# MolecularAI/GraphINVENT

Hardware: NVIDIA B200
Metric: molecular-graphs/sec (train fwd+bwd) GGNN (higher is better)
Workload: dtype f32

## Files before the change

graphinvent_b200/csrc/gemm.cuh:

```cuda
#pragma once
#include "common.cuh"
#include "prof.cuh"

namespace gib {

enum Epi : int {
  EPI_ACT = 0,
  EPI_MUL_DACT = 1,
  EPI_ADD = 2
};

struct GemmNT {
  const float* A = nullptr; int lda = 0;
  const float* B = nullptr; int ldb = 0;
  const float* B_hi = nullptr;
  const float* B_lo = nullptr;
  float* C = nullptr; int ldc = 0;
  int M = 0, N = 0, K = 0;
  const float* bias = nullptr;
  int act = ACT_NONE;
  int mode = EPI_ACT;
  const float* aux = nullptr; int ldaux = 0;
  int n_store = 0;
  int n_valid = 0;
  double work = 0;
  const int* m_dev = nullptr;
  const int* base_dev = nullptr;
};

struct GemmTN {
  const float* G; int ldg;
  const float* X; int ldx;
  int M, Nn, Kk, chunk_rows;
  float* ws; float* ws_bias;
};

struct GemmDW {
  const float* G = nullptr; int ldg = 0; int Nn = 0;
  const float* X = nullptr; int ldx = 0; int Kk = 0;
  int M = 0;
  float* dW = nullptr; float* dbias = nullptr;
  int R = 0, C = 0, Rb = 0, Rbp = 0;
  long long rs = 0, cs = 1;
  float* scratch = nullptr;
  size_t half_floats = 0;
  double work = 0;
  const int* m_dev = nullptr;
  const int* base_dev = nullptr;
};

constexpr int kTc3MaxProblems = 16;

struct Dw3Layout {
  int chunk_rows;
  int cap_splits[kTc3MaxProblems];
  size_t part_off[kTc3MaxProblems];
  size_t bias_off[kTc3MaxProblems];
  size_t floats;
};

int gemm_nt(const GemmNT& p, cudaStream_t st);
int gemm_nt_simt(const GemmNT& p, cudaStream_t st);
int gemm_nt_tc(const GemmNT& p, cudaStream_t st);
int gemm_nt_tc_group(const GemmNT* ps, int n, cudaStream_t st);
int gemm_nt_group(const GemmNT* ps, int n, cudaStream_t st);
bool gemm_nt_chain_ok(const GemmNT* ps, int n);
int gemm_nt_chain(const GemmNT* ps, const int* dep, int n, int* flags, cudaStream_t st);
bool tc_eligible(const GemmNT& p);
bool tc3_eligible(const GemmNT& p);
int gemm_nt_tc3_group(const GemmNT* ps, int n, cudaStream_t st);
size_t tc3_chain_flag_ints(const GemmNT* ps, int n);
int gemm_nt_tc3_chain(const GemmNT* ps, const int* dep, int n, int* flags, cudaStream_t st);
bool tc3_dw_eligible(const GemmDW& q);
int tc3_dw_chunk_rows(const GemmDW* qs, int n, long long plan_rows);
void tc3_dw_layout(const GemmDW* qs, int n, int chunk_rows, Dw3Layout* L);
int gemm_dw_tc3_partials(const GemmDW* qs, int n, const Dw3Layout& L, float* scratch, cudaStream_t st);
int gemm_dw_tc3_reduce(const GemmDW* qs, int n, const Dw3Layout& L, const float* scratch, cudaStream_t st);
int device_sm_count();
void tc3_set_trace(long long* buf, int tiles);
int tc_make_map(void* cu_tensor_map, const float* base, int rows, int cols, int ld, int box_rows, int mn_major);
extern bool g_use_tc;
extern int g_tc_debug;
extern long long* g_tc_timing;

enum tc_timing_slots {
  TS_TMA_WAIT_EMPTY = 0, TS_TMA_TOTAL, TS_MMA_WAIT_SPLIT, TS_MMA_WAIT_ACC, TS_MMA_TOTAL, TS_SPL_WAIT_RAW, TS_SPL_WORK,
  TS_SPL_TOTAL, TS_EPI_WAIT_ACC, TS_EPI_WORK, TS_EPI_TOTAL, TS_KERNEL_TOTAL, TS_ITEMS, TS_KBLOCKS, TS_LAUNCHES,
  TIMING_SLOTS = 16, TIMING_CTAS = 160
};

int gemm_dw(const GemmDW& q, cudaStream_t st);
int gemm_dw_group(const GemmDW* qs, int n, long long plan_rows, cudaStream_t st);
size_t gemm_dw_group_half_floats(const GemmDW* qs, int n, long long plan_rows);
int dw_begin();
void gemm_dw_plan(int M, int Nn, int Kk, int* splits, int* chunk);
void tc_dw_plan(int M, int Nn, int Kk, int* splits, int* chunk);
bool tc_dw_eligible(const GemmDW& q);
int gemm_dw_tc_partials(const GemmDW& q, int* splits_out, cudaStream_t st);
size_t gemm_dw_scratch_floats(int M, int Nn, int Kk);
size_t gemm_dw_half_floats(int M, int Nn, int Kk);
int dw_join(cudaStream_t st);

}
```

graphinvent_b200/csrc/gemm_simt.cu:

```cuda
#include <algorithm>
#include <mutex>

#include "gemm.cuh"
#include "ops.cuh"

namespace gib {

constexpr int BK = 16;
constexpr int kColsumSplits = 296;

template <int BM, int BN, int RM, int RN>
__global__ void __launch_bounds__(256, 2) sgemm_nt_kernel(const GemmNT p) {
  static_assert((BM / (4 * RM)) * (BN / (4 * RN)) == 256, "256 threads");
  __shared__ __align__(16) float As[2][BK][BM + 4];
  __shared__ __align__(16) float Bs[2][BK][BN + 4];

  const int tid = threadIdx.x;
  const int w = tid >> 5, l = tid & 31;
  const int ty = (w >> 1) * 4 + (l >> 3);
  const int tx = (w & 1) * 8 + (l & 7);
  const int m0 = blockIdx.y * BM, n0 = blockIdx.x * BN;

  constexpr int LA = BM / 64, LB = BN / 64;
  float4 ra[LA], rb[LB];
// ... 76 lines not shown
    }
    if (t + 1 < ntiles) sstore(buf ^ 1);
    __syncthreads();
  }

  const bool vec_c = (p.ldc & 3) == 0 && ((reinterpret_cast<uintptr_t>(p.C) & 15) == 0);
  const bool vec_x = p.aux && (p.ldaux & 3) == 0 && ((reinterpret_cast<uintptr_t>(p.aux) & 15) == 0);
#pragma unroll
  for (int a = 0; a < RM; ++a)
#pragma unroll
    for (int i = 0; i < 4; ++i) {
      const int m = m0 + ty * 4 + a * (BM / RM) + i;
      if (m >= p.M) continue;
#pragma unroll
      for (int b = 0; b < RN; ++b) {
        const int n = n0 + tx * 4 + b * (BN / RN);
        if (n >= p.n_store) continue;
        float v[4] = {acc[a][i][b][0], acc[a][i][b][1], acc[a][i][b][2], acc[a][i][b][3]};
        float x[4] = {0.f, 0.f, 0.f, 0.f};
        if (p.mode != EPI_ACT) {
          if (vec_x && n + 3 < p.n_store) {
            float4 t4 = *reinterpret_cast<const float4*>(p.aux + (size_t)m * p.ldaux + n);
            x[0] = t4.x; x[1] = t4.y; x[2] = t4.z; x[3] = t4.w;
          } else {
#pragma unroll
            for (int j = 0; j < 4; ++j)
              if (n + j < p.n_store) x[j] = p.aux[(size_t)m * p.ldaux + n + j];
          }
        }
#pragma unroll
        for (int j = 0; j < 4; ++j) {
          if (p.mode == EPI_ACT) {
            float bj = (p.bias && n + j < p.N) ? p.bias[n + j] : 0.f;
            v[j] = act_f(v[j] + bj, p.act);
          } else if (p.mode == EPI_MUL_DACT) {
            v[j] = v[j] * dact_from_out(x[j], p.act);
          } else {
            v[j] = v[j] + x[j];
          }
          if (n + j >= p.n_valid) v[j] = 0.f;
        }
        float* dst = p.C + (size_t)m * p.ldc + n;
        if (vec_c && n + 3 < p.n_store) {
          *reinterpret_cast<float4*>(dst) = make_float4(v[0], v[1], v[2], v[3]);
        } else {
#pragma unroll
          for (int j = 0; j < 4; ++j)
            if (n + j < p.n_store) dst[j] = v[j];
        }
      }
    }
}

static inline bool use_tc3() { return (g_tc_debug & 1) == 0; }

int gemm_nt(const GemmNT& p, cudaStream_t st) {
  if (p.m_dev) {
    if (!g_use_tc || !use_tc3() || !tc3_eligible(p)) {
      set_error("gemm_nt: device-side row counts need the tcgen05 path (tensor cores on, pre-split weights)");
      return -2;
    }
    return gemm_nt_tc3_group(&p, 1, st);
  }
  if (g_use_tc && p.N >= 48 && p.K >= 32) {
    if (use_tc3() && p.M >= 256 && tc3_eligible(p)) return gemm_nt_tc3_group(&p, 1, st);
    if (p.M >= 1024 && tc_eligible(p)) return gemm_nt_tc(p, st);
  }
  if (g_use_tc && use_tc3() && (g_tc_debug & 4) && p.N < 48 && p.K >= 128 && p.M >= 256 && tc3_eligible(p))
    return gemm_nt_tc3_group(&p, 1, st);
  return gemm_nt_simt(p, st);
}

int gemm_nt_group(const GemmNT* ps, int n, cudaStream_t st) {
  if (n == 1) return gemm_nt(ps[0], st);
  bool ok = g_use_tc && n <= 4, ok3 = ok && use_tc3(), dyn = false;
  long long tiles = 0;
  for (int i = 0; i < n && ok; ++i) {
    if (ps[i].m_dev) dyn = true;
    if (ps[i].M <= 0 || ps[i].N <= 0) continue;
    ok = tc_eligible(ps[i]) && ps[i].K >= 32 && ps[i].N >= 48;
    ok3 = ok3 && ok && tc3_eligible(ps[i]);
    tiles += (long long)ceil_div(ps[i].M, 128) * ceil_div(ps[i].N, 128);
  }
  if (ok3 && (tiles >= 4 || dyn)) return gemm_nt_tc3_group(ps, n, st);
  if (ok && !dyn && tiles >= 16) return gemm_nt_tc_group(ps, n, st);
  for (int i = 0; i < n; ++i) GIB_TRY(gemm_nt(ps[i], st));
  return 0;
}

bool gemm_nt_chain_ok(const GemmNT* ps, int n) {
  if (!g_use_tc || !use_tc3() || n < 2 || n > kTc3MaxProblems || (g_tc_debug & 2)) return false;
  long long tiles = 0;
  bool dyn = false;
  for (int i = 0; i < n; ++i) {
    const GemmNT& p = ps[i];
    if (p.M <= 0 || p.N <= 0) continue;
    if (!tc3_eligible(p) || p.N < 48 || p.K < 32) return false;
    if (p.m_dev) dyn = true;
    tiles += (long long)ceil_div(p.M, 128) * ceil_div(p.N, 128);
  }
  return dyn || tiles >= 16;
}
int gemm_nt_chain(const GemmNT* ps, const int* dep, int n, int* flags, cudaStream_t st) {
  return gemm_nt_tc3_chain(ps, dep, n, flags, st);
}

int gemm_nt_simt(const GemmNT& p, cudaStream_t st) {
  if (p.M <= 0 || p.N <= 0) return 0;
  if (p.K % BK != 0 || (p.lda & 3) || (p.ldb & 3) || p.K <= 0) {
    set_error("gemm_nt: K=%d lda=%d ldb=%d violate the padded-layout contract", p.K, p.lda, p.ldb);
    return -2;
  }
  ProfScope prof(PROF_GEMM_NT_SIMT, p.work > 0 ? p.work : 2.0 * p.M * (double)p.N * p.K, st);
  const long long ctas_big = (long long)ceil_div(p.M, 128) * ceil_div(p.N, 128);
  const int num_sms = device_sm_count();
  if (ctas_big >= num_sms && p.N > 64) {
    dim3 grid(ceil_div(p.N, 128), ceil_div(p.M, 128));
    sgemm_nt_kernel<128, 128, 2, 2><<<grid, 256, 0, st>>>(p);
  } else if (p.N <= 64 && (long long)ceil_div(p.M, 128) >= num_sms) {
    dim3 grid(ceil_div(p.N, 64), ceil_div(p.M, 128));
    sgemm_nt_kernel<128, 64, 2, 1><<<grid, 256, 0, st>>>(p);
  } else {
    dim3 grid(ceil_div(p.N, 64), ceil_div(p.M, 64));
    sgemm_nt_kernel<64, 64, 1, 1><<<grid, 256, 0, st>>>(p);
  }
  GIB_LAUNCH_CHECK();
  return 0;
}

template <int BM, int BN, int RM, int RN>
__global__ void __launch_bounds__(256, 2) sgemm_tn_splitk_kernel(const GemmTN p) {
  __shared__ __align__(16) float As[2][BK][BM + 4];
  __shared__ __align__(16) float Bs[2][BK][BN + 4];
  const int tid = threadIdx.x;
  const int w = tid >> 5, l = tid & 31;
  const int ty = (w >> 1) * 4 + (l >> 3);
  const int tx = (w & 1) * 8 + (l & 7);
  const int n0 = blockIdx.y * BM;
  const int k0 = blockIdx.x * BN;
  const int z = blockIdx.z;
  const int m_begin = z * p.chunk_rows;
  const int m_end = min(p.M, m_begin + p.chunk_rows);

  constexpr int LA = BM / 64, LB = BN / 64;
  float4 ra[LA], rb[LB];
  auto gload = [&](int m0) {
#pragma unroll
    for (int i = 0; i < LA; ++i) {
      int q = tid + i * 256, kk = q / (BM / 4), c = (q % (BM / 4)) * 4;
      bool ok = (m0 + kk) < m_end && (n0 + c) < p.Nn;
      ra[i] = ok ? __ldg(reinterpret_cast<const float4*>(p.G + (size_t)(m0 + kk) * p.ldg + n0 + c))
                 : make_float4(0, 0, 0, 0);
    }
#pragma unroll
    for (int i = 0; i < LB; ++i) {
      int q = tid + i * 256, kk = q / (BN / 4), c = (q % (BN / 4)) * 4;
      bool ok = (m0 + kk) < m_end && (k0 + c) < p.Kk;
      rb[i] = ok ? __ldg(reinterpret_cast<const float4*>(p.X + (size_t)(m0 + kk) * p.ldx + k0 + c))
                 : make_float4(0, 0, 0, 0);
    }
  };
  auto sstore = [&](int buf) {
#pragma unroll
    for (int i = 0; i < LA; ++i) {
      int q = tid + i * 256, kk = q / (BM / 4), c = (q % (BM / 4)) * 4;
      *reinterpret_cast<float4*>(&As[buf][kk][c]) = ra[i];
    }
#pragma unroll
    for (int i = 0; i < LB; ++i) {
// ... 21 lines not shown
    gload(m_begin);
    sstore(0);
  }
  __syncthreads();
  for (int t = 0; t < ntiles; ++t) {
    const int buf = t & 1;
    if (t + 1 < ntiles) gload(m_begin + (t + 1) * BK);
#pragma unroll
    for (int kk = 0; kk < BK; ++kk) {
      float4 fa[RM], fb[RN];
#pragma unroll
      for (int a = 0; a < RM; ++a)
        fa[a] = *reinterpret_cast<const float4*>(&As[buf][kk][ty * 4 + a * (BM / RM)]);
#pragma unroll
      for (int b = 0; b < RN; ++b)
        fb[b] = *reinterpret_cast<const float4*>(&Bs[buf][kk][tx * 4 + b * (BN / RN)]);
#pragma unroll
      for (int a = 0; a < RM; ++a) {
        const float av[4] = {fa[a].x, fa[a].y, fa[a].z, fa[a].w};
        if (do_bias) {
#pragma unroll
          for (int i = 0; i < 4; ++i) bacc[a][i] += av[i];
        }
#pragma unroll
        for (int b = 0; b < RN; ++b) {
          const float bv[4] = {fb[b].x, fb[b].y, fb[b].z, fb[b].w};
#pragma unroll
          for (int i = 0; i < 4; ++i)
#pragma unroll
            for (int j = 0; j < 4; ++j) acc[a][i][b][j] = fmaf(av[i], bv[j], acc[a][i][b][j]);
        }
      }
    }
    if (t + 1 < ntiles) sstore(buf ^ 1);
    __syncthreads();
  }

  float* out = p.ws + (size_t)z * p.Nn * p.Kk;
#pragma unroll
  for (int a = 0; a < RM; ++a)
#pragma unroll
    for (int i = 0; i < 4; ++i) {
      const int n = n0 + ty * 4 + a * (BM / RM) + i;
      if (n >= p.Nn) continue;
#pragma unroll
      for (int b = 0; b < RN; ++b) {
        const int k = k0 + tx * 4 + b * (BN / RN);
        if (k >= p.Kk) continue;
        *reinterpret_cast<float4*>(out + (size_t)n * p.Kk + k) =
            make_float4(acc[a][i][b][0], acc[a][i][b][1], acc[a][i][b][2], acc[a][i][b][3]);
      }
      if (do_bias && (l & 7) == 0) p.ws_bias[(size_t)z * p.Nn + n] = bacc[a][i];
    }
}

__global__ void __launch_bounds__(256) reduce_grads_kernel(const float* __restrict__ ws, int splits, int Nn, int Kk,
                                                           float* __restrict__ dW, int R, int C, int Rb, int Rbp,
                                                           long long rs, long long cs, int nblk_w,
                                                           const float* __restrict__ wsb, int bsplits,
                                                           float* __restrict__ db) {
  if ((int)blockIdx.x < nblk_w) {
    const long long idx = (long long)blockIdx.x * 256 + threadIdx.x;
    if (idx >= (long long)R * C) return;
    const int r = (int)(idx / C), c = (int)(idx % C);
    const int prow = (r / Rb) * Rbp + (r % Rb);
    const float* src = ws + (size_t)prow * Kk + c;
    const size_t stride = (size_t)Nn * Kk;
    float s = 0.f;
    int zi = 0;
    for (; zi + 8 <= splits; zi += 8) {
      float v[8];
#pragma unroll
      for (int u = 0; u < 8; ++u) v[u] = src[(size_t)(zi + u) * stride];
#pragma unroll
      for (int u = 0; u < 8; ++u) s += v[u];
    }
    for (; zi < splits; ++zi) s += src[(size_t)zi * stride];
    dW[r * rs + c * cs] += s;
  } else {
    __shared__ float sm[8][33];
    const int r = ((int)blockIdx.x - nblk_w) * 32 + (threadIdx.x & 31);
    const int wy = threadIdx.x >> 5;
    float s = 0.f;
    if (r < R) {
      const int prow = (r / Rb) * Rbp + (r % Rb);
      for (int zi = wy; zi < bsplits; zi += 8) s += wsb[(size_t)zi * Nn + prow];
    }
    sm[wy][threadIdx.x & 31] = s;
    __syncthreads();
    if (wy == 0 && r < R) {
      float t = 0.f;
      for (int k = 0; k < 8; ++k) t += sm[k][threadIdx.x];
      db[r] += t;
    }
  }
}

static int launch_reduce(const float* ws, int splits, const GemmDW& q, const float* wsb, int bsplits, cudaStream_t st) {
  const int nblk_w = q.dW ? (int)ceil_div_ll((long long)q.R * q.C, 256) : 0;
  const int nblk_b = q.dbias ? ceil_div(q.R, 32) : 0;
  if (nblk_w + nblk_b == 0) return 0;
  reduce_grads_kernel<<<nblk_w + nblk_b, 256, 0, st>>>(ws, splits, q.Nn, q.Kk, q.dW, q.R, q.C, q.Rb, q.Rbp, q.rs, q.cs,
                                                      nblk_w, wsb, bsplits, q.dbias);
  GIB_LAUNCH_CHECK();
  return 0;
}
// ... 39 lines not shown
}

struct DwSide {
  cudaStream_t side = nullptr;
  cudaEvent_t ev_tn[2], ev_done[2];
  bool done_valid[2] = {false, false};
  long long calls = 0;
  int pending = -1;
  int last = -1;
};
static DwSide g_dw[64];
static std::mutex g_dw_mu;

static int dw_side(DwSide** out) {
  int dev = 0;
  GIB_CUDA_TRY(cudaGetDevice(&dev));
  if (dev < 0 || dev >= 64) { set_error("device index %d out of range", dev); return -4; }
  std::lock_guard<std::mutex> lk(g_dw_mu);
  DwSide& d = g_dw[dev];
  if (!d.side) {
    GIB_CUDA_TRY(cudaStreamCreateWithFlags(&d.side, cudaStreamNonBlocking));
    for (int i = 0; i < 2; ++i) {
      GIB_CUDA_TRY(cudaEventCreateWithFlags(&d.ev_tn[i], cudaEventDisableTiming));
      GIB_CUDA_TRY(cudaEventCreateWithFlags(&d.ev_done[i], cudaEventDisableTiming));
    }
  }
  *out = &d;
  return 0;
}

int dw_begin() {
  DwSide* d;
  GIB_TRY(dw_side(&d));
  d->done_valid[0] = d->done_valid[1] = false;
  d->calls = 0; d->pending = -1; d->last = -1;
  return 0;
}

int dw_join(cudaStream_t st) {
  DwSide* d;
  GIB_TRY(dw_side(&d));
  if (d->last >= 0) {
    GIB_CUDA_TRY(cudaStreamWaitEvent(st, d->ev_done[d->last], 0));
    d->last = -1; d->pending = -1;
  }
  return 0;
}

size_t gemm_dw_half_floats(int M, int Nn, int Kk) {
  int splits, chunk, s2, c2;
  gemm_dw_plan(M, Nn, Kk, &splits, &chunk);
  tc_dw_plan(M, Nn, Kk, &s2, &c2);
  if (s2 > splits) splits = s2;
  size_t f = (((size_t)splits * Nn * Kk + (size_t)(splits > kColsumSplits ? splits : kColsumSplits) * Nn) + 63) & ~(size_t)63;
  GemmDW q; q.M = M; q.Nn = Nn; q.Kk = Kk;
  Dw3Layout L;
  tc3_dw_layout(&q, 1, tc3_dw_chunk_rows(&q, 1, 0), &L);
  return std::max(f, (L.floats + 63) & ~(size_t)63);
}

size_t gemm_dw_scratch_floats(int M, int Nn, int Kk) {
  return 2 * gemm_dw_half_floats(M, Nn, Kk);
}

size_t gemm_dw_group_half_floats(const GemmDW* qs, int n, long long plan_rows) {
  size_t f = 0;
  for (int i = 0; i < n; ++i) f = std::max(f, gemm_dw_half_floats(qs[i].M, qs[i].Nn, qs[i].Kk));
  Dw3Layout L;
  tc3_dw_layout(qs, n, tc3_dw_chunk_rows(qs, n, plan_rows), &L);
  return std::max(f, (L.floats + 63) & ~(size_t)63);
}

void gemm_dw_plan(int M, int Nn, int Kk, int* splits, int* chunk) {
  const int tiles = ceil_div(Nn, 128) * ceil_div(Kk, 128);
  int s = ceil_div(2 * device_sm_count(), tiles);
  const int max_s = ceil_div(M, 64) > 0 ? ceil_div(M, 64) : 1;
  if (s > max_s) s = max_s;
  if (s < 1) s = 1;
  int c = ceil_div(ceil_div(M, s), BK) * BK;
  if (c < BK) c = BK;
  s = ceil_div(M, c);
  if (s < 1) s = 1;
  *splits = s;
  *chunk = c;
}

int gemm_dw_group(const GemmDW* qs, int n, long long plan_rows, cudaStream_t st) {
  if (n < 1) return 0;
  if (n > kTc3MaxProblems) { set_error("gemm_dw_group: %d problems (max %d)", n, kTc3MaxProblems); return -2; }
  const bool tc3 = g_use_tc && use_tc3();
  bool dyn = false;
  long long rows = 0;
  double work = 0;
  GemmDW live[kTc3MaxProblems];
  GemmDW rest[kTc3MaxProblems];
  int nl = 0, nr = 0;
  for (int i = 0; i < n; ++i) {
    const GemmDW& q = qs[i];
    if (q.M <= 0) continue;
    const bool good = tc3 && tc3_dw_eligible(q) && q.Nn >= 32 && q.Kk >= 32 && q.scratch == qs[0].scratch &&
                      q.half_floats == qs[0].half_floats;
    if (q.m_dev) {
      dyn = true;
      if (!good) {
        set_error("gemm_dw_group: device-side row counts need the tcgen05 path (tensor cores on, aligned operands)");
        return -2;
// ... 3 lines not shown
      rows += q.M;
      work += q.work > 0 ? q.work : 2.0 * q.M * (double)q.R * q.C;
      live[nl++] = q;
    } else {
      rest[nr++] = q;
    }
  }
  if (nl && !dyn && rows < 2048) {
    for (int i = 0; i < nl; ++i) rest[nr++] = live[i];
    nl = 0;
  }
  for (int i = 0; i < nr; ++i) GIB_TRY(gemm_dw(rest[i], st));
  if (nl == 0) return 0;
  ProfScope prof(PROF_GEMM_DW, work, st);
  DwSide* d;
  GIB_TRY(dw_side(&d));
  const int half = (int)(d->calls++ & 1);
  float* const scratch = live[0].scratch + (size_t)half * live[0].half_floats;
  Dw3Layout L;
  tc3_dw_layout(live, nl, tc3_dw_chunk_rows(qs, n, plan_rows), &L);
  if (L.floats > live[0].half_floats) {
    set_error("gemm_dw_group: scratch half of %zu floats is too small for %zu", live[0].half_floats, L.floats);
    return -2;
  }
  if (d->pending >= 0) {
    GIB_CUDA_TRY(cudaStreamWaitEvent(st, d->ev_done[d->pending], 0));
    d->pending = -1;
  }
  if (d->done_valid[half]) GIB_CUDA_TRY(cudaStreamWaitEvent(st, d->ev_done[half], 0));
  GIB_TRY(gemm_dw_tc3_partials(live, nl, L, scratch, st));
  GIB_CUDA_TRY(cudaEventRecord(d->ev_tn[half], st));
  GIB_CUDA_TRY(cudaStreamWaitEvent(d->side, d->ev_tn[half], 0));
  GIB_TRY(gemm_dw_tc3_reduce(live, nl, L, scratch, d->side));
  GIB_CUDA_TRY(cudaEventRecord(d->ev_done[half], d->side));
  d->done_valid[half] = true;
  d->last = half;
  return 0;
}

int gemm_dw(const GemmDW& q, cudaStream_t st) {
  if (q.M <= 0) return 0;
  if ((q.ldg & 3) || (q.ldx & 3) || (q.Nn & 3) || (q.Kk & 3)) {
    set_error("gemm_dw: ldg=%d ldx=%d Nn=%d Kk=%d violate the padded-layout contract", q.ldg, q.ldx, q.Nn, q.Kk);
    return -2;
  }
  if (q.m_dev || (g_use_tc && use_tc3() && q.dW && q.M >= 2048 && q.Nn >= 32 && q.Kk >= 32 && tc3_dw_eligible(q) &&
                  q.half_floats > 0))
    return gemm_dw_group(&q, 1, 0, st);
  ProfScope prof(g_use_tc && !use_tc3() ? PROF_GEMM_DW : PROF_GEMM_DW_SIMT, q.work > 0 ? q.work : 2.0 * q.M * (double)q.R * q.C, st);
  DwSide* d;
  GIB_TRY(dw_side(&d));
  const int half = (int)(d->calls++ & 1);
  float* const scratch = q.scratch + (size_t)half * q.half_floats;
  if (d->done_valid[half]) GIB_CUDA_TRY(cudaStreamWaitEvent(st, d->ev_done[half], 0));
  if (g_use_tc && q.dW && tc_dw_eligible(q)) {
    int tsplits = 0;
    GemmDW q2 = q;
    q2.scratch = scratch;
    GIB_TRY(gemm_dw_tc_partials(q2, &tsplits, st));
    GIB_CUDA_TRY(cudaEventRecord(d->ev_tn[half], st));
    GIB_CUDA_TRY(cudaStreamWaitEvent(d->side, d->ev_tn[half], 0));
    float* part = scratch + (size_t)tsplits * q.Nn * q.Kk;
    if (q.dbias) {
      colsum_partial_kernel<<<kColsumSplits, 256, 0, d->side>>>(part, q.G, q.ldg, q.M, q.Nn);
      GIB_LAUNCH_CHECK();
    }
    GIB_TRY(launch_reduce(scratch, tsplits, q, part, kColsumSplits, d->side));
    GIB_CUDA_TRY(cudaEventRecord(d->ev_done[half], d->side));
    d->done_valid[half] = true;
    const int prev = d->pending;
    d->pending = half;
    d->last = half;
    if (prev >= 0 && prev != half) GIB_CUDA_TRY(cudaStreamWaitEvent(st, d->ev_done[prev], 0));
    return 0;
  }
  GIB_TRY(dw_join(st));
  int splits, chunk;
  gemm_dw_plan(q.M, q.Nn, q.Kk, &splits, &chunk);
  GemmTN p;
  p.G = q.G; p.ldg = q.ldg; p.X = q.X; p.ldx = q.ldx; p.M = q.M; p.Nn = q.Nn; p.Kk = q.Kk;
  p.chunk_rows = chunk;
  p.ws = scratch;
  p.ws_bias = q.dbias ? scratch + (size_t)splits * q.Nn * q.Kk : nullptr;
  if (q.dW) {
    dim3 grid(ceil_div(q.Kk, 128), ceil_div(q.Nn, 128), splits);
    sgemm_tn_splitk_kernel<128, 128, 2, 2><<<grid, 256, 0, st>>>(p);
    GIB_LAUNCH_CHECK();
  } else if (q.dbias) {
    GemmTN pb = p;
    pb.Kk = 4;
    dim3 grid(1, ceil_div(q.Nn, 128), splits);
    sgemm_tn_splitk_kernel<128, 128, 2, 2><<<grid, 256, 0, st>>>(pb);
    GIB_LAUNCH_CHECK();
  }
  GIB_TRY(launch_reduce(p.ws, splits, q, p.ws_bias, splits, st));
  return 0;
}

}
```

graphinvent_b200/csrc/model.cu:

```cuda
#include <vector>

#include "../../include/gib200.h"
#include "gemm.cuh"
#include "model.cuh"
#include "ops.cuh"

namespace gib {

static void finish_lin(Plan& pl, Lin& l) {
  l.Rbp = pad16(l.Rb);
  l.Rp = l.nblk * l.Rbp;
  l.Cp = pad16(l.C);
  l.Ctp = pad16(l.Ct);
  l.ow = pl.packed_floats;  pl.packed_floats += (size_t)l.Rp * l.Cp;
  l.owt = pl.packed_floats; pl.packed_floats += (size_t)l.Ctp * l.Rp;
  l.ob = pl.packed_floats;  pl.packed_floats += (size_t)l.Rp;
  pl.packed_floats = (pl.packed_floats + 31) & ~(size_t)31;
  l.ow_hi = pl.packed_floats;  pl.packed_floats += (size_t)l.Rp * l.Cp;
  l.ow_lo = pl.packed_floats;  pl.packed_floats += (size_t)l.Rp * l.Cp;
  l.owt_hi = pl.packed_floats; pl.packed_floats += (size_t)l.Ctp * l.Rp;
  l.owt_lo = pl.packed_floats; pl.packed_floats += (size_t)l.Ctp * l.Rp;
  pl.packed_floats = (pl.packed_floats + 31) & ~(size_t)31;
}

// ... 288 lines not shown
    q.G = G; q.ldg = L.Rp; q.Nn = L.Rp;
    q.X = Xin; q.ldx = ldxin; q.Kk = L.Cp;
    q.M = rows;
    q.dW = r.grads[L.pw] + L.src_off;
    q.dbias = L.pb >= 0 ? r.grads[L.pb] : nullptr;
    q.R = L.R; q.C = L.C; q.Rb = L.Rb; q.Rbp = L.Rbp; q.rs = L.rs; q.cs = L.cs;
    q.scratch = r.scratch + bb.dw; q.half_floats = bb.dw_half;
    q.work = 2.0 * rows * (double)L.R * L.C;
    GIB_TRY(gemm_dw(q, r.st));
    if (l > 1 || dX0) {
      GemmNT p;
      p.A = G; p.lda = L.Rp;
      p.B = r.packed + L.owt; p.ldb = L.Rp; p.B_hi = r.packed + L.owt_hi; p.B_lo = r.packed + L.owt_lo;
      p.M = rows; p.N = L.Ctp; p.K = L.Rp;
      p.n_store = L.Ctp; p.n_valid = L.Ctp;
      p.work = 2.0 * rows * (double)L.R * L.Ct;
      if (l > 1) {
        p.C = (G == ping) ? pong : ping; p.ldc = L.Ctp;
        p.mode = EPI_MUL_DACT; p.act = m.act;
        p.aux = Xin; p.ldaux = ldxin;
      } else {
        p.C = dX0; p.ldc = ld_dx;
        if (dx_aux) { p.mode = EPI_ADD; p.aux = dx_aux; p.ldaux = ld_dx; }
        else { p.mode = EPI_ACT; p.act = ACT_NONE; p.bias = nullptr; }
      }
      GIB_TRY(gemm_nt(p, r.st));
      G = p.C;
    }
  }
  if (m.n == 1) GIB_TRY(dw_join(r.st));
  return 0;
}

struct MlpJob {
  const Mlp* m; const float* X0; const MlpAct* a; long long row0; int rows;
  float* ext_out; int ext_ld, ext_valid;
  const int* m_dev = nullptr; const int* base_dev = nullptr;
};
struct MlpBwdJob {
  const Mlp* m; const float* X0; const MlpAct* a; long long row0; int rows;
  const float* Gtop; float* dX0; int ld_dx; const float* dx_aux;
  const int* m_dev = nullptr; const int* base_dev = nullptr;
};
static int* fwd_flags(const Run& r) { return reinterpret_cast<int*>(r.ws + r.L.flags); }
static const int* type_count_dev(const Run& r, int g) { return r.cap ? r.dev_hdr + HDR_TYPE_COUNT + g : nullptr; }
static const int* type_base_dev(const Run& r, int g) { return r.cap ? r.dev_hdr + HDR_TYPE_BASE + g : nullptr; }

static size_t mlp_max_ld(const Plan& pl, const Mlp& m) {
  size_t w = 16;
  for (int l = 0; l < m.n; ++l) w = std::max(w, (size_t)std::max(pl.lins[m.first + l].Rp, pl.lins[m.first + l].Cp));
  return w;
}

static int mlp_forward_multi(const Run& r, const MlpJob* jobs, int n, int* flags = nullptr) {
  bool same = n <= 4;
  for (int i = 1; i < n && same; ++i) same = jobs[i].m->n == jobs[0].m->n;
  if (!same) {
    for (int i = 0; i < n; ++i) {
      if (jobs[i].m_dev) { set_error("mlp_forward_multi: device-side row counts need MLPs of equal depth"); return -2; }
      GIB_TRY(mlp_forward(r, *jobs[i].m, jobs[i].X0, *jobs[i].a, jobs[i].row0, jobs[i].rows, jobs[i].ext_out,
                          jobs[i].ext_ld, jobs[i].ext_valid));
    }
    return 0;
  }
  const float* x[4]; int ldx[4];
  for (int i = 0; i < n; ++i) { x[i] = jobs[i].X0 + (size_t)jobs[i].row0 * jobs[i].a->ld[0]; ldx[i] = jobs[i].a->ld[0]; }
  const int depth = jobs[0].m->n;
  GemmNT all[kTc3MaxProblems];
  int dep[kTc3MaxProblems], layer_of[kTc3MaxProblems], last[4] = {-1, -1, -1, -1}, nall = 0;
  const bool try_chain = depth >= 2 && depth * n <= kTc3MaxProblems;
  for (int l = 1; l <= depth; ++l) {
    GemmNT ps[4];
    int np = 0, idx[4];
    for (int i = 0; i < n; ++i) {
      const MlpJob& j = jobs[i];
      if (j.rows <= 0) continue;
      const Lin& L = r.pl.lins[j.m->first + l - 1];
      GemmNT& p = ps[np];
      p = GemmNT();
      p.A = x[i]; p.lda = ldx[i];
      p.B = r.packed + L.ow; p.ldb = L.Cp; p.B_hi = r.packed + L.ow_hi; p.B_lo = r.packed + L.ow_lo;
      p.M = j.rows; p.N = L.Rp; p.K = L.Cp;
      p.bias = L.pb >= 0 ? r.packed + L.ob : nullptr;
      p.act = j.m->act; p.mode = EPI_ACT;
      p.work = 2.0 * j.rows * (double)L.R * L.C;
      p.m_dev = j.m_dev; p.base_dev = j.base_dev;
      if (l == j.m->n && j.ext_out) {
        p.C = j.ext_out + (size_t)j.row0 * j.ext_ld; p.ldc = j.ext_ld; p.n_store = j.ext_valid; p.n_valid = j.ext_valid;
      } else {
        p.C = r.ws + j.a->y[l] + (size_t)j.row0 * j.a->ld[l]; p.ldc = j.a->ld[l]; p.n_store = L.Rp; p.n_valid = L.Rp;
      }
      if (ldx[i] < L.Cp) { set_error("mlp_forward_multi: input ld %d < padded K %d", ldx[i], L.Cp); return -2; }
      idx[np++] = i;
    }
    if (try_chain) {
      for (int k = 0; k < np; ++k) {
        all[nall] = ps[k];
        dep[nall] = last[idx[k]];
        layer_of[nall] = l;
        last[idx[k]] = nall++;
      }
    } else {
      GIB_TRY(gemm_nt_group(ps, np, r.st));
    }
    for (int k = 0; k < np; ++k) { x[idx[k]] = ps[k].C; ldx[idx[k]] = ps[k].ldc; }
  }
  if (try_chain && nall) {
    if (flags && gemm_nt_chain_ok(all, nall)) return gemm_nt_chain(all, dep, nall, flags, r.st);
    int k0 = 0;
    if (flags) {
      int k = nall;
      while (k > 0 && layer_of[k - 1] >= 3) {
        const int l = layer_of[k - 1];
        while (k > 0 && layer_of[k - 1] == l) --k;
        if (gemm_nt_chain_ok(all, k)) {
          GIB_TRY(gemm_nt_chain(all, dep, k, flags, r.st));
          k0 = k;
          break;
        }
      }
    }
    while (k0 < nall) {
      int k1 = k0 + 1;
      while (k1 < nall && layer_of[k1] == layer_of[k0]) ++k1;
      GIB_TRY(gemm_nt_group(all + k0, k1 - k0, r.st));
      k0 = k1;
    }
  }
  return 0;
}

static int mlp_backward_multi(const Run& r, const BwdBufs& bb, const MlpBwdJob* jobs, int n, long long plan_rows = 0) {
  bool same = n <= 4;
  for (int i = 1; i < n && same; ++i) same = jobs[i].m->n == jobs[0].m->n;
  const int depth = jobs[0].m->n;
  if (!same || depth > 8 || depth * n > kTc3MaxProblems) {
    for (int i = 0; i < n; ++i) {
      if (jobs[i].m_dev) { set_error("mlp_backward_multi: device-side row counts need MLPs of equal depth"); return -2; }
      GIB_TRY(mlp_backward(r, bb, *jobs[i].m, jobs[i].X0, *jobs[i].a, jobs[i].row0, jobs[i].rows, jobs[i].Gtop,
                           jobs[i].dX0, jobs[i].ld_dx, jobs[i].dx_aux));
    }
    return 0;
  }
  const float* G[9][4];
  size_t off = 0;
  for (int i = 0; i < n; ++i) {
    G[depth][i] = jobs[i].Gtop;
    for (int l = 1; l < depth; ++l) G[l][i] = r.scratch + bb.Gl[l] + off;
    if (!jobs[i].m_dev) off += ((size_t)std::max(jobs[i].rows, 0) * mlp_max_ld(r.pl, *jobs[i].m) + 31) & ~(size_t)31;
  }
  auto x_in = [&](const MlpBwdJob& j, int l, int* ld) -> const float* {
    *ld = j.a->ld[l - 1];
    return (l == 1) ? j.X0 + (size_t)j.row0 * j.a->ld[0] : r.ws + j.a->y[l - 1] + (size_t)j.row0 * j.a->ld[l - 1];
  };
  GemmNT all[kTc3MaxProblems];
  int dep[kTc3MaxProblems], layer_of[kTc3MaxProblems], last[4] = {-1, -1, -1, -1}, nall = 0;
  for (int l = depth; l >= 2; --l)
    for (int i = 0; i < n; ++i) {
      const MlpBwdJob& j = jobs[i];
      if (j.rows <= 0) continue;
      const Lin& L = r.pl.lins[j.m->first + l - 1];
      int ldxin;
      const float* Xin = x_in(j, l, &ldxin);
      GemmNT& p = all[nall];
      p = GemmNT();
      p.A = G[l][i]; p.lda = L.Rp; p.B = r.packed + L.owt; p.ldb = L.Rp;
      p.B_hi = r.packed + L.owt_hi; p.B_lo = r.packed + L.owt_lo;
      p.M = j.rows; p.N = L.Ctp; p.K = L.Rp; p.n_store = L.Ctp; p.n_valid = L.Ctp;
      p.work = 2.0 * j.rows * (double)L.R * L.Ct;
      p.C = const_cast<float*>(G[l - 1][i]); p.ldc = L.Ctp;
      p.mode = EPI_MUL_DACT; p.act = j.m->act; p.aux = Xin; p.ldaux = ldxin;
      p.m_dev = j.m_dev; p.base_dev = j.base_dev;
      dep[nall] = last[i];
      layer_of[nall] = l;
      last[i] = nall++;
    }
  if (nall) {
    int k0 = 0;
    while (k0 < nall) {
      if (nall - k0 >= 2 && gemm_nt_chain_ok(all + k0, nall - k0)) {
        int dep2[kTc3MaxProblems];
        for (int k = k0; k < nall; ++k) dep2[k - k0] = dep[k] >= k0 ? dep[k] - k0 : -1;
        GIB_TRY(gemm_nt_chain(all + k0, dep2, nall - k0, reinterpret_cast<int*>(r.scratch + bb.flags), r.st));
        break;
      }
      int k1 = k0 + 1;
      while (k1 < nall && layer_of[k1] == layer_of[k0]) ++k1;
      GIB_TRY(gemm_nt_group(all + k0, k1 - k0, r.st));
      k0 = k1;
    }
  }
  for (int i = 0; i < n; ++i) {
    const MlpBwdJob& j = jobs[i];
    if (j.rows <= 0 || !j.dX0) continue;
    const Lin& L = r.pl.lins[j.m->first];
    GemmNT p1;
    p1.A = G[1][i]; p1.lda = L.Rp; p1.B = r.packed + L.owt; p1.ldb = L.Rp;
    p1.B_hi = r.packed + L.owt_hi; p1.B_lo = r.packed + L.owt_lo;
    p1.M = j.rows; p1.N = L.Ctp; p1.K = L.Rp; p1.n_store = L.Ctp; p1.n_valid = L.Ctp;
    p1.work = 2.0 * j.rows * (double)L.R * L.Ct;
    p1.C = j.dX0; p1.ldc = j.ld_dx;
    p1.m_dev = j.m_dev; p1.base_dev = j.base_dev;
    if (j.dx_aux) { p1.mode = EPI_ADD; p1.aux = j.dx_aux; p1.ldaux = j.ld_dx; }
    else { p1.mode = EPI_ACT; p1.act = ACT_NONE; p1.bias = nullptr; }
    GIB_TRY(gemm_nt(p1, r.st));
  }
  GemmDW qs[kTc3MaxProblems];
  int nq = 0;
  for (int l = depth; l >= 1; --l)
    for (int i = 0; i < n; ++i) {
      const MlpBwdJob& j = jobs[i];
      if (j.rows <= 0) continue;
      const Lin& L = r.pl.lins[j.m->first + l - 1];
      int ldxin;
      const float* Xin = x_in(j, l, &ldxin);
      GemmDW& q = qs[nq++];
      q = GemmDW();
      q.G = G[l][i]; q.ldg = L.Rp; q.Nn = L.Rp; q.X = Xin; q.ldx = ldxin; q.Kk = L.Cp; q.M = j.rows;
      q.dW = r.grads[L.pw] + L.src_off;
      q.dbias = L.pb >= 0 ? r.grads[L.pb] : nullptr;
      q.R = L.R; q.C = L.C; q.Rb = L.Rb; q.Rbp = L.Rbp; q.rs = L.rs; q.cs = L.cs;
      q.scratch = r.scratch + bb.dw; q.half_floats = bb.dw_half;
      q.work = 2.0 * j.rows * (double)L.R * L.C;
      q.m_dev = j.m_dev; q.base_dev = j.base_dev;
    }
  GIB_TRY(gemm_dw_group(qs, nq, plan_rows * depth, r.st));
  if (!(g_use_tc && (g_tc_debug & 1) == 0)) GIB_TRY(dw_join(r.st));
  return 0;
}

static int readout_forward(const Run& r, float* out) {
  const gib_dims& d = r.pl.d;
  const Plan& pl = r.pl;
  const Layout& L = r.L;
  const long long S = r.S;
  const int Hp = pl.Hp, Gp = pl.Gp;
// ... 469 lines not shown
```

Baseline: 265,100.

## Add narrow-N and small-K SIMT kernels and chain tensor-core GEMMs around them

```diff
diff --git a/graphinvent_b200/csrc/gemm.cuh b/graphinvent_b200/csrc/gemm.cuh
--- a/graphinvent_b200/csrc/gemm.cuh
+++ b/graphinvent_b200/csrc/gemm.cuh
@@ -65,6 +65,7 @@
 int gemm_nt_tc_group(const GemmNT* ps, int n, cudaStream_t st);
 int gemm_nt_group(const GemmNT* ps, int n, cudaStream_t st);
 bool gemm_nt_chain_ok(const GemmNT* ps, int n);
+bool gemm_nt_chain_member_ok(const GemmNT& p);
 int gemm_nt_chain(const GemmNT* ps, const int* dep, int n, int* flags, cudaStream_t st);
 bool tc_eligible(const GemmNT& p);
 bool tc3_eligible(const GemmNT& p);
diff --git a/graphinvent_b200/csrc/gemm_simt.cu b/graphinvent_b200/csrc/gemm_simt.cu
--- a/graphinvent_b200/csrc/gemm_simt.cu
+++ b/graphinvent_b200/csrc/gemm_simt.cu
@@ -152,6 +152,137 @@
     }
 }
 
+constexpr int kNarrowThreads = 128;
+
+template <int NP>
+__global__ void __launch_bounds__(kNarrowThreads) narrow_nt_kernel(const GemmNT p) {
+  constexpr int R = 32 / NP;
+  extern __shared__ float4 Bs4[];
+  const int K4 = p.K >> 2;
+  for (int i = threadIdx.x; i < NP * K4; i += kNarrowThreads) {
+    const int n = i / K4, q = i - n * K4;
+    Bs4[i] = n < p.N ? __ldg(reinterpret_cast<const float4*>(p.B + (size_t)n * p.ldb) + q) : make_float4(0, 0, 0, 0);
+  }
+  __syncthreads();
+  const int lane = threadIdx.x & 31;
+  const int nwarps = gridDim.x * (kNarrowThreads / 32);
+  for (int m0 = (blockIdx.x * (kNarrowThreads / 32) + (threadIdx.x >> 5)) * R; m0 < p.M; m0 += nwarps * R) {
+    float v[32];
+#pragma unroll
+    for (int i = 0; i < 32; ++i) v[i] = 0.f;
+    const float* arow[R];
+#pragma unroll
+    for (int r = 0; r < R; ++r) arow[r] = p.A + (size_t)min(m0 + r, p.M - 1) * p.lda;
+#pragma unroll 4
+    for (int q = lane; q < K4; q += 32) {
+      float4 a[R];
+#pragma unroll
+      for (int r = 0; r < R; ++r) a[r] = __ldg(reinterpret_cast<const float4*>(arow[r]) + q);
+#pragma unroll
+      for (int n = 0; n < NP; ++n) {
+        const float4 b = Bs4[n * K4 + q];
+#pragma unroll
+        for (int r = 0; r < R; ++r) {
+          float& s = v[r * NP + n];
+          s = fmaf(a[r].x, b.x, s); s = fmaf(a[r].y, b.y, s); s = fmaf(a[r].z, b.z, s); s = fmaf(a[r].w, b.w, s);
+        }
+      }
+    }
+#pragma unroll
+    for (int w = 16; w >= 1; w >>= 1) {
+      const bool up = (lane & w) != 0;
+#pragma unroll
+      for (int i = 0; i < w; ++i) {
+        const float send = up ? v[i] : v[i + w];
+        const float keep = up ? v[i + w] : v[i];
+        v[i] = keep + __shfl_xor_sync(0xffffffffu, send, w);
+      }
+    }
+    const int m = m0 + lane / NP, n = lane % NP;
+    if (m >= p.M || n >= p.n_store) continue;
+    float y = v[0];
+    if (p.mode == EPI_ACT) y = act_f(y + ((p.bias && n < p.N) ? p.bias[n] : 0.f), p.act);
+    else if (p.mode == EPI_MUL_DACT) y *= dact_from_out(p.aux[(size_t)m * p.ldaux + n], p.act);
+    else y += p.aux[(size_t)m * p.ldaux + n];
+    p.C[(size_t)m * p.ldc + n] = n < p.n_valid ? y : 0.f;
+  }
+}
+
+constexpr int kSmallKThreads = 128;
+
+__device__ __forceinline__ void smallk_row(const GemmNT& p, const float (&w)[4][16], int m, int n, bool vec_c,
+                                           bool vec_x) {
+  const float4* a4 = reinterpret_cast<const float4*>(p.A + (size_t)m * p.lda);
+  float a[16];
+#pragma unroll
+  for (int i = 0; i < 4; ++i) {
+    const float4 t = __ldg(a4 + i);
+    a[4 * i] = t.x; a[4 * i + 1] = t.y; a[4 * i + 2] = t.z; a[4 * i + 3] = t.w;
+  }
+  float x[4] = {0.f, 0.f, 0.f, 0.f};
+  if (p.mode != EPI_ACT) {
+    if (vec_x && n + 3 < p.n_store) {
+      const float4 t = __ldg(reinterpret_cast<const float4*>(p.aux + (size_t)m * p.ldaux + n));
+      x[0] = t.x; x[1] = t.y; x[2] = t.z; x[3] = t.w;
+    } else {
+#pragma unroll
+      for (int j = 0; j < 4; ++j)
+        if (n + j < p.n_store) x[j] = p.aux[(size_t)m * p.ldaux + n + j];
+    }
+  }
+  float v[4];
+#pragma unroll
+  for (int j = 0; j < 4; ++j) {
+    float s = 0.f;
+#pragma unroll
+    for (int k = 0; k < 16; ++k) s = fmaf(a[k], w[j][k], s);
+    if (p.mode == EPI_ACT) s = act_f(s + ((p.bias && n + j < p.N) ? p.bias[n + j] : 0.f), p.act);
+    else if (p.mode == EPI_MUL_DACT) s *= dact_from_out(x[j], p.act);
+    else s += x[j];
+    v[j] = n + j < p.n_valid ? s : 0.f;
+  }
+  float* dst = p.C + (size_t)m * p.ldc + n;
+  if (vec_c && n + 3 < p.n_store) {
+    *reinterpret_cast<float4*>(dst) = make_float4(v[0], v[1], v[2], v[3]);
+  } else {
+#pragma unroll
+    for (int j = 0; j < 4; ++j)
+      if (n + j < p.n_store) dst[j] = v[j];
+  }
+}
+
+__global__ void __launch_bounds__(kSmallKThreads) smallk_nt_kernel(const GemmNT p) {
+  const int n = (blockIdx.y * kSmallKThreads + threadIdx.x) * 4;
+  if (n >= p.n_store) return;
+  float w[4][16];
+#pragma unroll
+  for (int j = 0; j < 4; ++j)
+#pragma unroll
+    for (int i = 0; i < 4; ++i) {
+      const float4 t = n + j < p.N ? __ldg(reinterpret_cast<const float4*>(p.B + (size_t)(n + j) * p.ldb) + i)
+                                   : make_float4(0, 0, 0, 0);
+      w[j][4 * i] = t.x; w[j][4 * i + 1] = t.y; w[j][4 * i + 2] = t.z; w[j][4 * i + 3] = t.w;
+    }
+  const bool vec_c = (p.ldc & 3) == 0 && ((reinterpret_cast<uintptr_t>(p.C) & 15) == 0);
+  const bool vec_x = p.aux && (p.ldaux & 3) == 0 && ((reinterpret_cast<uintptr_t>(p.aux) & 15) == 0);
+  const int stride = 2 * gridDim.x;
+  int m = 2 * blockIdx.x;
+  for (; m + 1 < p.M; m += stride) {
+    smallk_row(p, w, m, n, vec_c, vec_x);
+    smallk_row(p, w, m + 1, n, vec_c, vec_x);
+  }
+  if (m < p.M) smallk_row(p, w, m, n, vec_c, vec_x);
+}
+
+static bool narrow_nt_ok(const GemmNT& p) {
+  const int w = std::max(p.N, p.n_store);
+  return w <= 32 && (size_t)(w <= 16 ? 16 : 32) * p.K * sizeof(float) <= 48 * 1024 &&
+         (reinterpret_cast<uintptr_t>(p.A) & 15) == 0 && (reinterpret_cast<uintptr_t>(p.B) & 15) == 0;
+}
+static bool smallk_nt_ok(const GemmNT& p) {
+  return p.K == 16 && (reinterpret_cast<uintptr_t>(p.A) & 15) == 0 && (reinterpret_cast<uintptr_t>(p.B) & 15) == 0;
+}
+
 static inline bool use_tc3() { return (g_tc_debug & 1) == 0; }
 
 int gemm_nt(const GemmNT& p, cudaStream_t st) {
@@ -188,6 +319,9 @@
   return 0;
 }
 
+bool gemm_nt_chain_member_ok(const GemmNT& p) {
+  return p.M <= 0 || p.N <= 0 || (tc3_eligible(p) && p.N >= 48 && p.K >= 32);
+}
 bool gemm_nt_chain_ok(const GemmNT* ps, int n) {
   if (!g_use_tc || !use_tc3() || n < 2 || n > kTc3MaxProblems || (g_tc_debug & 2)) return false;
   long long tiles = 0;
@@ -195,7 +329,7 @@
   for (int i = 0; i < n; ++i) {
     const GemmNT& p = ps[i];
     if (p.M <= 0 || p.N <= 0) continue;
-    if (!tc3_eligible(p) || p.N < 48 || p.K < 32) return false;
+    if (!gemm_nt_chain_member_ok(p)) return false;
     if (p.m_dev) dyn = true;
     tiles += (long long)ceil_div(p.M, 128) * ceil_div(p.N, 128);
   }
@@ -214,7 +348,16 @@
   ProfScope prof(PROF_GEMM_NT_SIMT, p.work > 0 ? p.work : 2.0 * p.M * (double)p.N * p.K, st);
   const long long ctas_big = (long long)ceil_div(p.M, 128) * ceil_div(p.N, 128);
   const int num_sms = device_sm_count();
-  if (ctas_big >= num_sms && p.N > 64) {
+  if (narrow_nt_ok(p)) {
+    const int np = std::max(p.N, p.n_store) <= 16 ? 16 : 32, rows_per_cta = (kNarrowThreads / 32) * (32 / np);
+    const int grid = (int)std::min<long long>(ceil_div(p.M, rows_per_cta), 6LL * num_sms);
+    if (np == 16) narrow_nt_kernel<16><<<grid, kNarrowThreads, (size_t)16 * p.K * sizeof(float), st>>>(p);
+    else narrow_nt_kernel<32><<<grid, kNarrowThreads, (size_t)32 * p.K * sizeof(float), st>>>(p);
+  } else if (smallk_nt_ok(p)) {
+    const int col_blocks = ceil_div(ceil_div(p.n_store, 4), kSmallKThreads);
+    dim3 grid((unsigned)std::min<long long>(ceil_div(p.M, 2), std::max(1, 8 * num_sms / col_blocks)), col_blocks);
+    smallk_nt_kernel<<<grid, kSmallKThreads, 0, st>>>(p);
+  } else if (ctas_big >= num_sms && p.N > 64) {
     dim3 grid(ceil_div(p.N, 128), ceil_div(p.M, 128));
     sgemm_nt_kernel<128, 128, 2, 2><<<grid, 256, 0, st>>>(p);
   } else if (p.N <= 64 && (long long)ceil_div(p.M, 128) >= num_sms) {
@@ -342,6 +485,86 @@
       }
       if (do_bias && (l & 7) == 0) p.ws_bias[(size_t)z * p.Nn + n] = bacc[a][i];
     }
+}
+
+constexpr int kNarrowDwGroups = 4, kNarrowDwQuads = 128;
+constexpr size_t kNarrowDwSmem = (size_t)(kNarrowDwGroups - 1) * 16 * kNarrowDwQuads * sizeof(float4) +
+                                 (size_t)kNarrowDwGroups * 16 * sizeof(float);
+
+__global__ void __launch_bounds__(kNarrowDwGroups * kNarrowDwQuads) narrow_dw_kernel(const GemmTN p) {
+  extern __shared__ float4 red[];
+  float* redb = reinterpret_cast<float*>(red + (kNarrowDwGroups - 1) * 16 * kNarrowDwQuads);
+  const int t = threadIdx.x % kNarrowDwQuads, g = threadIdx.x / kNarrowDwQuads;
+  const int k = (blockIdx.y * kNarrowDwQuads + t) * 4;
+  const bool kok = k < p.Kk;
+  const int z = blockIdx.x;
+  const int m_begin = z * p.chunk_rows, m_end = min(p.M, m_begin + p.chunk_rows);
+  const int n4 = p.Nn >> 2;
+  const bool do_bias = p.ws_bias != nullptr && blockIdx.y == 0 && t == 0;
+  float4 acc[16];
+  float bacc[16];
+#pragma unroll
+  for (int n = 0; n < 16; ++n) { acc[n] = make_float4(0.f, 0.f, 0.f, 0.f); bacc[n] = 0.f; }
+  for (int m = m_begin + g; m < m_end; m += kNarrowDwGroups) {
+    const float4 x = kok ? __ldg(reinterpret_cast<const float4*>(p.X + (size_t)m * p.ldx + k)) : make_float4(0, 0, 0, 0);
+    const float4* g4 = reinterpret_cast<const float4*>(p.G + (size_t)m * p.ldg);
+    float gv[16];
+#pragma unroll
+    for (int i = 0; i < 4; ++i) {
+      const float4 u = i < n4 ? __ldg(g4 + i) : make_float4(0, 0, 0, 0);
+      gv[4 * i] = u.x; gv[4 * i + 1] = u.y; gv[4 * i + 2] = u.z; gv[4 * i + 3] = u.w;
+    }
+#pragma unroll
+    for (int n = 0; n < 16; ++n) {
+      acc[n].x = fmaf(gv[n], x.x, acc[n].x); acc[n].y = fmaf(gv[n], x.y, acc[n].y);
+      acc[n].z = fmaf(gv[n], x.z, acc[n].z); acc[n].w = fmaf(gv[n], x.w, acc[n].w);
+    }
+    if (do_bias) {
+#pragma unroll
+      for (int n = 0; n < 16; ++n) bacc[n] += gv[n];
+    }
+  }
+  if (g > 0) {
+#pragma unroll
+    for (int n = 0; n < 16; ++n) red[((g - 1) * 16 + n) * kNarrowDwQuads + t] = acc[n];
+  }
+  if (do_bias) {
+#pragma unroll
+    for (int n = 0; n < 16; ++n) redb[g * 16 + n] = bacc[n];
+  }
+  __syncthreads();
+  if (g != 0) return;
+  for (int h = 1; h < kNarrowDwGroups; ++h) {
+#pragma unroll
+    for (int n = 0; n < 16; ++n) {
+      const float4 u = red[((h - 1) * 16 + n) * kNarrowDwQuads + t];
+      acc[n].x += u.x; acc[n].y += u.y; acc[n].z += u.z; acc[n].w += u.w;
+    }
+  }
+  if (kok) {
+    float* out = p.ws + (size_t)z * p.Nn * p.Kk + k;
+#pragma unroll
+    for (int n = 0; n < 16; ++n)
+      if (n < p.Nn) *reinterpret_cast<float4*>(out + (size_t)n * p.Kk) = acc[n];
+  }
+  if (do_bias) {
+    for (int n = 0; n < p.Nn; ++n) {
+      float s = redb[n];
+      for (int h = 1; h < kNarrowDwGroups; ++h) s += redb[h * 16 + n];
+      p.ws_bias[(size_t)z * p.Nn + n] = s;
+    }
+  }
+}
+
+static void narrow_dw_plan(int M, int* splits, int* chunk) {
+  int s = std::max(1, std::min(ceil_div(M, 16), device_sm_count()));
+  const int c = ceil_div(M, s);
+  *splits = ceil_div(M, c);
+  *chunk = c;
+}
+static bool narrow_dw_ok(const GemmDW& q) {
+  return q.dW && q.Nn <= 16 && (q.ldg & 3) == 0 && (q.ldx & 3) == 0 && (reinterpret_cast<uintptr_t>(q.G) & 15) == 0 &&
+         (reinterpret_cast<uintptr_t>(q.X) & 15) == 0;
 }
 
 __global__ void __launch_bounds__(256) reduce_grads_kernel(const float* __restrict__ ws, int splits, int Nn, int Kk,
@@ -487,6 +710,10 @@
   gemm_dw_plan(M, Nn, Kk, &splits, &chunk);
   tc_dw_plan(M, Nn, Kk, &s2, &c2);
   if (s2 > splits) splits = s2;
+  if (Nn <= 16) {
+    narrow_dw_plan(M, &s2, &c2);
+    if (s2 > splits) splits = s2;
+  }
   size_t f = (((size_t)splits * Nn * Kk + (size_t)(splits > kColsumSplits ? splits : kColsumSplits) * Nn) + 63) & ~(size_t)63;
   GemmDW q; q.M = M; q.Nn = Nn; q.Kk = Kk;
   Dw3Layout L;
@@ -596,6 +823,43 @@
   GIB_TRY(dw_side(&d));
   const int half = (int)(d->calls++ & 1);
   float* const scratch = q.scratch + (size_t)half * q.half_floats;
+  if (narrow_dw_ok(q)) {
+    int splits, chunk;
+    narrow_dw_plan(q.M, &splits, &chunk);
+    const size_t per_split = (size_t)q.Nn * q.Kk + q.Nn;
+    if ((size_t)splits * per_split > q.half_floats) {
+      splits = std::max<long long>(1, (long long)(q.half_floats / per_split));
+      chunk = ceil_div(q.M, splits);
+      splits = ceil_div(q.M, chunk);
+    }
+    static bool smem_set[64] = {false};
+    int dev = 0;
+    GIB_CUDA_TRY(cudaGetDevice(&dev));
+    if (!smem_set[dev & 63]) {
+      GIB_CUDA_TRY(cudaFuncSetAttribute(narrow_dw_kernel, cudaFuncAttributeMaxDynamicSharedMemorySize, (int)kNarrowDwSmem));
+      smem_set[dev & 63] = true;
+    }
+    if (d->pending >= 0) {
+      GIB_CUDA_TRY(cudaStreamWaitEvent(st, d->ev_done[d->pending], 0));
+      d->pending = -1;
+    }
+    if (d->done_valid[half]) GIB_CUDA_TRY(cudaStreamWaitEvent(st, d->ev_done[half], 0));
+    GemmTN p;
+    p.G = q.G; p.ldg = q.ldg; p.X = q.X; p.ldx = q.ldx; p.M = q.M; p.Nn = q.Nn; p.Kk = q.Kk;
+    p.chunk_rows = chunk;
+    p.ws = scratch;
+    p.ws_bias = q.dbias ? scratch + (size_t)splits * q.Nn * q.Kk : nullptr;
+    dim3 grid(splits, ceil_div(ceil_div(q.Kk, 4), kNarrowDwQuads));
+    narrow_dw_kernel<<<grid, kNarrowDwGroups * kNarrowDwQuads, kNarrowDwSmem, st>>>(p);
+    GIB_LAUNCH_CHECK();
+    GIB_CUDA_TRY(cudaEventRecord(d->ev_tn[half], st));
+    GIB_CUDA_TRY(cudaStreamWaitEvent(d->side, d->ev_tn[half], 0));
+    GIB_TRY(launch_reduce(p.ws, splits, q, p.ws_bias, splits, d->side));
+    GIB_CUDA_TRY(cudaEventRecord(d->ev_done[half], d->side));
+    d->done_valid[half] = true;
+    d->last = half;
+    return 0;
+  }
   if (d->done_valid[half]) GIB_CUDA_TRY(cudaStreamWaitEvent(st, d->ev_done[half], 0));
   if (g_use_tc && q.dW && tc_dw_eligible(q)) {
     int tsplits = 0;
diff --git a/graphinvent_b200/csrc/model.cu b/graphinvent_b200/csrc/model.cu
--- a/graphinvent_b200/csrc/model.cu
+++ b/graphinvent_b200/csrc/model.cu
@@ -364,6 +364,40 @@
   return w;
 }
 
+static int chain_around_narrow(const Run& r, const GemmNT* all, const int* dep, int nall, int* flags) {
+  if (!flags || nall > kTc3MaxProblems) return 0;
+  bool before[kTc3MaxProblems], after[kTc3MaxProblems], needed[kTc3MaxProblems];
+  int idx[kTc3MaxProblems], cdep[kTc3MaxProblems], nn = 0;
+  GemmNT chain[kTc3MaxProblems];
+  for (int i = 0; i < nall; ++i) needed[i] = false;
+  for (int i = 0; i < nall; ++i)
+    if (dep[i] >= 0) needed[dep[i]] = true;
+  for (int i = 0; i < nall; ++i) {
+    const bool narrow = !gemm_nt_chain_member_ok(all[i]);
+    before[i] = narrow && (dep[i] < 0 || before[dep[i]]);
+    after[i] = narrow && !before[i] && !needed[i];
+    if (narrow && !before[i] && !after[i]) return 0;
+    nn += narrow;
+  }
+  if (nn == 0) return 0;
+  int nc = 0;
+  for (int i = 0; i < nall; ++i) {
+    idx[i] = -1;
+    if (before[i] || after[i]) continue;
+    idx[i] = nc;
+    chain[nc] = all[i];
+    cdep[nc] = dep[i] >= 0 ? idx[dep[i]] : -1;
+    ++nc;
+  }
+  if (!gemm_nt_chain_ok(chain, nc)) return 0;
+  for (int i = 0; i < nall; ++i)
+    if (before[i]) GIB_TRY(gemm_nt(all[i], r.st));
+  GIB_TRY(gemm_nt_chain(chain, cdep, nc, flags, r.st));
+  for (int i = 0; i < nall; ++i)
+    if (after[i]) GIB_TRY(gemm_nt(all[i], r.st));
+  return 1;
+}
+
 static int mlp_forward_multi(const Run& r, const MlpJob* jobs, int n, int* flags = nullptr) {
   bool same = n <= 4;
   for (int i = 1; i < n && same; ++i) same = jobs[i].m->n == jobs[0].m->n;
@@ -419,6 +453,8 @@
   }
   if (try_chain && nall) {
     if (flags && gemm_nt_chain_ok(all, nall)) return gemm_nt_chain(all, dep, nall, flags, r.st);
+    const int rc = chain_around_narrow(r, all, dep, nall, flags);
+    if (rc) return rc < 0 ? rc : 0;
     int k0 = 0;
     if (flags) {
       int k = nall;
@@ -488,12 +524,15 @@
       last[i] = nall++;
     }
   if (nall) {
-    int k0 = 0;
+    int* const flags = reinterpret_cast<int*>(r.scratch + bb.flags);
+    int k0 = gemm_nt_chain_ok(all, nall) ? 0 : chain_around_narrow(r, all, dep, nall, flags);
+    if (k0 < 0) return k0;
+    k0 = k0 ? nall : 0;
     while (k0 < nall) {
       if (nall - k0 >= 2 && gemm_nt_chain_ok(all + k0, nall - k0)) {
         int dep2[kTc3MaxProblems];
         for (int k = k0; k < nall; ++k) dep2[k - k0] = dep[k] >= k0 ? dep[k] - k0 : -1;
-        GIB_TRY(gemm_nt_chain(all + k0, dep2, nall - k0, reinterpret_cast<int*>(r.scratch + bb.flags), r.st));
+        GIB_TRY(gemm_nt_chain(all + k0, dep2, nall - k0, flags, r.st));
         break;
       }
       int k1 = k0 + 1;
```

Result: faster. 274,200, median of 6 (+3.4%).
